# ZulutionAI/MoviiGen1.1

Measured on AMD Instinct MI355X. Metric: denoise-steps/sec, higher is better.
Workload: dtype bf16; 1 GPU; 14B T2V 1920x832x81f bf16 (the metric's configuration; BASELINE configs[2] shape); layers=40, parallelism=single, solver=unipc, weights=random N(0,0.02) bf16, seed 0

## Files before the change

moviigen1.1_amd/csrc/attn_hd128_m16.hip:

```cpp
#include <type_traits>
#include "common.h"
#include "../../include/moviigen_hip.h"

#define M16_THREADS 256
#define M16_QB 256
#define M16_TILE 16384
#define M16_K(slot) ((slot) * M16_TILE)
#define M16_V(slot) (3 * M16_TILE + (slot) * M16_TILE)

MG_DEV bf16x8_t m16_bf(u32x4_t v) { return __builtin_bit_cast(bf16x8_t, v); }
struct M16State {
    f32x4_t ot[8][4];
    f32x4_t st[2][2][4];
    bf16x8_t pf[2][4];
    f32x4_t mq[4];
    float m_run[4], l_run[4];
    float psa[4], psb[4];
    int bad;
};

template <int OFF>
MG_DEV void m16_rd(bf16x8_t& dst, unsigned addr) {
    asm volatile("ds_read_b128 %0, %1 offset:%2" : "=v"(dst) : "v"(addr), "i"(OFF));
}
template <int N>
MG_DEV void m16_wait() {
    asm volatile("s_waitcnt lgkmcnt(%0)" ::"i"(N) : "memory");
}
MG_DEV void m16_mfma_s0(f32x4_t& acc, const bf16x8_t& a, const bf16x8_t& b, const f32x4_t& c) {
    asm volatile("v_mfma_f32_16x16x32_bf16 %0, %1, %2, %3" : "=&v"(acc) : "v"(a), "a"(b), "v"(c));
}
MG_DEV void m16_mfma_s(f32x4_t& acc, const bf16x8_t& a, const bf16x8_t& b) {
    asm volatile("v_mfma_f32_16x16x32_bf16 %0, %1, %2, %0" : "+v"(acc) : "v"(a), "a"(b));
}
MG_DEV void m16_mfma_s_after_valu(f32x4_t& acc, const bf16x8_t& a, const bf16x8_t& b) {
    asm volatile("s_nop 7\n\ts_nop 7\n\tv_mfma_f32_16x16x32_bf16 %0, %1, %2, %0" : "+v"(acc) : "v"(a), "a"(b));
}
constexpr int m16_koff(int i) { return (i >> 2) * 256 + (i & 3) * 4096; }
constexpr int m16_voff(int i) { return i * 256; }

template <int KB>
MG_DEV void m16_softmax_exact(M16State& s, float c) {
#pragma unroll
    for (int n = 0; n < 4; ++n) {
        float tmax = s.st[KB][0][n][0];
#pragma unroll
        for (int r = 1; r < 4; ++r) tmax = fmaxf(tmax, s.st[KB][0][n][r]);
#pragma unroll
        for (int r = 0; r < 4; ++r) tmax = fmaxf(tmax, s.st[KB][1][n][r]);
        tmax = fmaxf(tmax, __shfl_xor(tmax, 16, 64));
        tmax = fmaxf(tmax, __shfl_xor(tmax, 32, 64));
        const float m_new = fmaxf(s.m_run[n], tmax);
        float psum = 0.f;
        float p[8];
#pragma unroll
        for (int r = 0; r < 8; ++r) {
            p[r] = __builtin_amdgcn_exp2f((s.st[KB][r >> 2][n][r & 3] - m_new) * c);
            psum += p[r];
        }
        u32x4_t w;
#pragma unroll
        for (int e = 0; e < 4; ++e) w[e] = pack_bf2(p[2 * e], p[2 * e + 1]);
        s.pf[KB][n] = m16_bf(w);
        const float alpha = __builtin_amdgcn_exp2f((s.m_run[n] - m_new) * c);
        s.l_run[n] = s.l_run[n] * alpha + psum;
#pragma unroll
        for (int d = 0; d < 8; ++d)
#pragma unroll
            for (int e = 0; e < 4; ++e) s.ot[d][n][e] *= alpha;
        s.m_run[n] = m_new;
    }
}

template <int KB>
MG_DEV void m16_softmax_zero(M16State& s, float c) {
#pragma unroll
    for (int n = 0; n < 4; ++n) {
        float psum = 0.f;
        float p[8];
#pragma unroll
        for (int r = 0; r < 8; ++r) {
            p[r] = __builtin_amdgcn_exp2f(s.st[KB][r >> 2][n][r & 3] * c);
            psum += p[r];
        }
        u32x4_t w;
#pragma unroll
        for (int e = 0; e < 4; ++e) w[e] = pack_bf2(p[2 * e], p[2 * e + 1]);
        s.pf[KB][n] = m16_bf(w);
        s.l_run[n] += psum;
    }
}

template <int KB>
MG_DEV void m16_mask_init(M16State& s, int lim, int G, const f32x4_t (&base)[4]) {
#pragma unroll
    for (int blk = 0; blk < 2; ++blk)
#pragma unroll
        for (int n = 0; n < 4; ++n)
#pragma unroll
            for (int r = 0; r < 4; ++r) {
                const int key = KB * 32 + G * 8 + blk * 4 + r;
                s.st[KB][blk][n][r] = key >= lim ? -1e30f : base[n][0];
            }
}

template <int KB, int SMODE, bool PV, bool SM, bool SCALED, int ORD, int LKO = 0, int LVO = 0, int NKO = 0, int NVO = 0, typename Dma>
MG_DEV void m16_step(M16State& s, const bf16x8_t (&qf)[4][4], bf16x8_t (&kf)[4], bf16x8_t (&vf)[4], unsigned lds_k,
                     unsigned lds_v, unsigned nk, unsigned nv, float c, Dma dma) {
    constexpr int SB = 1 - KB;
    u32x4_t w[4];
    float pa[2] = {0.f, 0.f}, pb[2] = {0.f, 0.f};
    auto exp_a = [&](int i, int half) __attribute__((always_inline)) {
        if (SM) {
            const int pp = 2 * i + half, n = pp >> 2, wd = pp & 3;
            const float x = s.st[SB][wd >> 1][n][(wd & 1) * 2];
            pa[half] = __builtin_amdgcn_exp2f(SCALED ? x * c : x);
            asm volatile("" : "+v"(pa[half]));
        }
    };
    auto exp_b = [&](int i, int half) __attribute__((always_inline)) {
        if (SM) {
            const int pp = 2 * i + half, n = pp >> 2, wd = pp & 3;
            const float x = s.st[SB][wd >> 1][n][(wd & 1) * 2 + 1];
            pb[half] = __builtin_amdgcn_exp2f(SCALED ? x * c : x);
            asm volatile("" : "+v"(pb[half]));
        }
    };
    auto add_a = [&](int i, int half) __attribute__((always_inline)) {
        if (SM) {
            const int n = (2 * i + half) >> 2;
            s.psa[n] += pa[half];
            asm volatile("" : "+v"(s.psa[n]));
        }
    };
    auto add_b = [&](int i, int half) __attribute__((always_inline)) {
        if (SM) {
            const int n = (2 * i + half) >> 2;
            s.psb[n] += pb[half];
            asm volatile("" : "+v"(s.psb[n]));
        }
    };
    auto cvt = [&](int i, int half) __attribute__((always_inline)) {
        if (SM) {
            const int pp = 2 * i + half, n = pp >> 2, wd = pp & 3;
            unsigned pk = pack_bf2(pa[half], pb[half]);
            asm volatile("" : "+v"(pk));
            w[n][wd] = pk;
        }
    };
    auto S = [&](int i, int n) __attribute__((always_inline)) {
        const int blk = i >> 2, c = i & 3, r = i & 3;
        if (SMODE == 1 && c == 0) m16_mfma_s0(s.st[KB][blk][n], kf[r], qf[n][c], s.mq[n]);
        else if (SMODE == 2 && c == 0) m16_mfma_s_after_valu(s.st[KB][blk][n], kf[r], qf[n][c]);
        else if (SMODE != 0) m16_mfma_s(s.st[KB][blk][n], kf[r], qf[n][c]);
    };
    auto P = [&](int i, int n) __attribute__((always_inline)) {
        if (PV) s.ot[i][n] = __builtin_amdgcn_mfma_f32_16x16x32_bf16(vf[i & 3], s.pf[KB][n], s.ot[i][n], 0, 0, 0);
    };
    auto rdK = [&](int i) __attribute__((always_inline)) {
        const int r2 = (i + 2) & 3;
        if (SMODE == 0) asm volatile("" ::"v"(kf[r2]));
        if (i < 6) {
            switch (i) {
                case 0: m16_rd<m16_koff(2) + LKO>(kf[r2], lds_k); break;
                case 1: m16_rd<m16_koff(3) + LKO>(kf[r2], lds_k); break;
                case 2: m16_rd<m16_koff(4) + LKO>(kf[r2], lds_k); break;
                case 3: m16_rd<m16_koff(5) + LKO>(kf[r2], lds_k); break;
                case 4: m16_rd<m16_koff(6) + LKO>(kf[r2], lds_k); break;
                default: m16_rd<m16_koff(7) + LKO>(kf[r2], lds_k); break;
            }
        } else if (i == 6) m16_rd<m16_koff(0) + NKO>(kf[r2], nk);
        else m16_rd<m16_koff(1) + NKO>(kf[r2], nk);
    };
    auto rdV = [&](int i) __attribute__((always_inline)) {
        const int r2 = (i + 2) & 3;
        if (i < 6) {
            switch (i) {
                case 0: m16_rd<m16_voff(2) + LVO>(vf[r2], lds_v); break;
                case 1: m16_rd<m16_voff(3) + LVO>(vf[r2], lds_v); break;
                case 2: m16_rd<m16_voff(4) + LVO>(vf[r2], lds_v); break;
                case 3: m16_rd<m16_voff(5) + LVO>(vf[r2], lds_v); break;
                case 4: m16_rd<m16_voff(6) + LVO>(vf[r2], lds_v); break;
                default: m16_rd<m16_voff(7) + LVO>(vf[r2], lds_v); break;
            }
        } else if (i == 6) m16_rd<m16_voff(0) + NVO>(vf[r2], nv);
        else m16_rd<m16_voff(1) + NVO>(vf[r2], nv);
    };
#define M16_SB() __builtin_amdgcn_sched_barrier(0)
#pragma unroll
    for (int i = 0; i < 8; ++i) {
        m16_wait<2>();
        M16_SB();
        if constexpr (ORD == 0) {
            S(i, 0); M16_SB();
            exp_a(i, 0); exp_b(i, 0); M16_SB();
            P(i, 0); M16_SB();
            add_a(i, 0); add_b(i, 0); cvt(i, 0); M16_SB();
            S(i, 1); M16_SB();
            rdK(i); M16_SB();
            P(i, 1); M16_SB();
            rdV(i); M16_SB();
            S(i, 2); M16_SB();
            exp_a(i, 1); exp_b(i, 1); M16_SB();
            P(i, 2); M16_SB();
            add_a(i, 1); add_b(i, 1); cvt(i, 1); M16_SB();
            S(i, 3); M16_SB();
            dma(i); M16_SB();
            P(i, 3); M16_SB();
        } else if constexpr (ORD == 1) {
            S(i, 0); M16_SB();
            exp_a(i, 0); M16_SB();
            P(i, 0); M16_SB();
            exp_b(i, 0); M16_SB();
            S(i, 1); M16_SB();
            add_a(i, 0); add_b(i, 0); cvt(i, 0); M16_SB();
            P(i, 1); M16_SB();
            rdK(i); M16_SB(); rdV(i); M16_SB();
            S(i, 2); M16_SB();
            exp_a(i, 1); M16_SB();
            P(i, 2); M16_SB();
            exp_b(i, 1); M16_SB();
            S(i, 3); M16_SB();
            add_a(i, 1); add_b(i, 1); cvt(i, 1); M16_SB();
            P(i, 3); M16_SB();
            dma(i); M16_SB();
        } else if constexpr (ORD == 2) {
            S(i, 0); M16_SB();
            exp_a(i, 0); M16_SB(); rdK(i); M16_SB();
            P(i, 0); M16_SB();
            exp_b(i, 0); M16_SB(); rdV(i); M16_SB();
            S(i, 1); M16_SB();
            add_a(i, 0); add_b(i, 0); cvt(i, 0); M16_SB();
            P(i, 1); M16_SB();
            S(i, 2); M16_SB();
            exp_a(i, 1); M16_SB();
            P(i, 2); M16_SB();
            exp_b(i, 1); M16_SB();
            S(i, 3); M16_SB();
            add_a(i, 1); add_b(i, 1); cvt(i, 1); M16_SB();
            P(i, 3); M16_SB();
            dma(i); M16_SB();
        } else if constexpr (ORD == 4) {
            S(i, 0); M16_SB();
            exp_a(i, 0); M16_SB();
            P(i, 0); M16_SB();
            exp_b(i, 0); M16_SB();
            S(i, 1); M16_SB();
            add_a(i, 0); add_b(i, 0); M16_SB();
            P(i, 1); M16_SB();
            cvt(i, 0); M16_SB(); rdK(i); M16_SB(); rdV(i); M16_SB();
            S(i, 2); M16_SB();
            exp_a(i, 1); M16_SB();
            P(i, 2); M16_SB();
            exp_b(i, 1); M16_SB();
            S(i, 3); M16_SB();
            add_a(i, 1); add_b(i, 1); M16_SB();
            P(i, 3); M16_SB();
            cvt(i, 1); M16_SB(); dma(i); M16_SB();
        } else if constexpr (ORD == 5) {
            S(i, 0); M16_SB();
            exp_a(i, 0); M16_SB();
            P(i, 0); M16_SB();
            exp_b(i, 0); M16_SB();
            S(i, 1); M16_SB();
            add_a(i, 0); add_b(i, 0); cvt(i, 0); M16_SB();
            P(i, 1); M16_SB();
            rdK(i); M16_SB();
            S(i, 2); M16_SB();
            exp_a(i, 1); M16_SB();
            P(i, 2); M16_SB();
            exp_b(i, 1); M16_SB();
            S(i, 3); M16_SB();
            add_a(i, 1); add_b(i, 1); cvt(i, 1); M16_SB();
            P(i, 3); M16_SB();
            rdV(i); M16_SB(); dma(i); M16_SB();
        } else if constexpr (ORD == 8) {
            S(i, 0); M16_SB();
            exp_a(i, 0); M16_SB();
            S(i, 1); M16_SB();
            exp_b(i, 0); M16_SB();
            P(i, 0); M16_SB();
            add_a(i, 0); add_b(i, 0); cvt(i, 0); M16_SB();
            P(i, 1); M16_SB();
            rdK(i); M16_SB(); rdV(i); M16_SB();
            S(i, 2); M16_SB();
            exp_a(i, 1); M16_SB();
            S(i, 3); M16_SB();
            exp_b(i, 1); M16_SB();
            P(i, 2); M16_SB();
            add_a(i, 1); add_b(i, 1); cvt(i, 1); M16_SB();
            P(i, 3); M16_SB();
            dma(i); M16_SB();
        } else if constexpr (ORD == 9) {
            S(i, 0); M16_SB();
            exp_a(i, 0); M16_SB();
            S(i, 1); M16_SB();
            exp_b(i, 0); M16_SB();
            S(i, 2); M16_SB();
            add_a(i, 0); add_b(i, 0); cvt(i, 0); M16_SB();
            S(i, 3); M16_SB();
            rdK(i); M16_SB(); rdV(i); M16_SB();
            P(i, 0); M16_SB();
            exp_a(i, 1); M16_SB();
            P(i, 1); M16_SB();
            exp_b(i, 1); M16_SB();
            P(i, 2); M16_SB();
            add_a(i, 1); add_b(i, 1); cvt(i, 1); M16_SB();
            P(i, 3); M16_SB();
            dma(i); M16_SB();
        } else {
            S(i, 0); M16_SB();
            exp_a(i, 0); M16_SB();
            P(i, 0); M16_SB();
            exp_b(i, 0); M16_SB();
            S(i, 1); M16_SB();
            exp_a(i, 1); M16_SB();
            P(i, 1); M16_SB();
            exp_b(i, 1); M16_SB();
            S(i, 2); M16_SB();
            add_a(i, 0); add_b(i, 0); cvt(i, 0); M16_SB();
            P(i, 2); M16_SB();
            add_a(i, 1); add_b(i, 1); cvt(i, 1); M16_SB();
            S(i, 3); M16_SB();
            rdK(i); M16_SB(); rdV(i); M16_SB();
            P(i, 3); M16_SB();
            dma(i); M16_SB();
        }
    }
#undef M16_SB
    if (SM) {
#pragma unroll
        for (int n = 0; n < 4; ++n) {
            s.pf[SB][n] = m16_bf(w[n]);
        }
    }
}

MG_DEV int m16_lane() {
    int l;
    asm volatile("v_mbcnt_lo_u32_b32 %0, -1, 0\n\tv_mbcnt_hi_u32_b32 %0, -1, %0" : "=v"(l));
    return l;
}

struct M16NoDma {
    __device__ __forceinline__ void operator()(int) const {}
};

template <bool PROF, bool SCALED, int ORD>
__global__ __launch_bounds__(M16_THREADS, 1) void attn_hd128_m16_kernel(
    const uint16_t* __restrict__ q, int64_t ldq, const uint16_t* __restrict__ kp, const uint16_t* __restrict__ vp,
    uint16_t* __restrict__ o, int64_t ldo, int64_t Lq, int64_t Lk, int heads, float c_log2, int nqb, int dbg,
    unsigned long long* __restrict__ prof, float* __restrict__ lse, unsigned* __restrict__ flagcnt, unsigned* __restrict__ tickets) {
    __shared__ __attribute__((aligned(16))) char smem[6 * M16_TILE];
    __shared__ int s_next_item;
    const int bid = blockIdx.x;
    const unsigned long long r_start = PROF ? __builtin_amdgcn_s_memrealtime() : 0;
    const int tid = threadIdx.x;
    const int wave = __builtin_amdgcn_readfirstlane(tid >> 6);
    const int total_items = nqb * heads;
    const int nwg = gridDim.x;
    const bool ticketed = tickets != nullptr && nwg != total_items;
    int item, item_end, item_step;
    if (nwg == total_items || ticketed) {
        item = bid, item_end = ticketed ? total_items : bid + 1, item_step = 1;
    } else {
        const int xcd = bid & 7, slot = bid >> 3;
        item = (int)((int64_t)xcd * total_items / 8) + slot;
        item_end = (int)((int64_t)(xcd + 1) * total_items / 8);
        item_step = nwg >> 3;
    }
    unsigned next_ticket = 0;
    unsigned long long ph[8] = {0, 0, 0, 0, 0, 0, 0, 0}, ph_t = 0;
    unsigned long long pf_fence = 0, pf_a = 0, pf_b = 0, pf_n = 0;
    while (item < item_end) {
    if (ticketed && tid == 0) next_ticket = atomicAdd(tickets, 1u);
    const int head = item / nqb;
    const int qb0 = item - head * nqb;
    const int lane = m16_lane();
    int qi = lane & 15, G = lane >> 4;
    __syncthreads();
    if (PROF) ph_t = __builtin_amdgcn_s_memtime();

    bf16x8_t qf[4][4];
    const int64_t qrow_base = (int64_t)qb0 * M16_QB + wave * 64 + qi;
#pragma unroll
    for (int n = 0; n < 4; ++n) {
        const int64_t qr = qrow_base + n * 16;
        const int64_t qrow = qr < Lq ? qr : Lq - 1;
        const uint16_t* qp = q + qrow * ldq + head * 128 + G * 8;
#pragma unroll
        for (int c = 0; c < 4; ++c) qf[n][c] = m16_bf(*(const u32x4_t*)(qp + c * 32));
    }
    const int T = (int)((Lk + 63) / 64);
    const int last_lim = (int)(Lk - (int64_t)(T - 1) * 64);
    const int nfull = last_lim == 64 ? T : T - 1;
    const unsigned lds0 = (unsigned)(uintptr_t)(mg_lptr_t)smem;
    const uint64_t kb64 = (uint64_t)(uintptr_t)(kp + ((int64_t)head * T) * 8192), vb64 = (uint64_t)(uintptr_t)(vp + ((int64_t)head * T) * 8192);
    const u32x4_t rs_k = {(unsigned)__builtin_amdgcn_readfirstlane((int)(unsigned)kb64), (unsigned)__builtin_amdgcn_readfirstlane((int)((unsigned)(kb64 >> 32) & 0xffffu)),
                          (unsigned)T * M16_TILE, 0x00020000u};
    const u32x4_t rs_v = {(unsigned)__builtin_amdgcn_readfirstlane((int)(unsigned)vb64), (unsigned)__builtin_amdgcn_readfirstlane((int)((unsigned)(vb64 >> 32) & 0xffffu)),
                          (unsigned)T * M16_TILE, 0x00020000u};
    const int dvo = wave * 4096 + lane * 16;
    const unsigned lds_w = (unsigned)__builtin_amdgcn_readfirstlane((int)(lds0 + wave * 4096));
    auto dma_tile4 = [&](const u32x4_t& rs, int t, unsigned lbase) __attribute__((always_inline)) {
        const int soff = __builtin_amdgcn_readfirstlane((t < T ? t : T - 1) * M16_TILE);
        asm volatile("s_mov_b32 m0, %2\n\ts_nop 4\n\t"
                     "buffer_load_dwordx4 %0, %1, %3 offen lds\n\t"
                     "buffer_load_dwordx4 %0, %1, %3 offen offset:1024 lds\n\t"
                     "buffer_load_dwordx4 %0, %1, %3 offen offset:2048 lds\n\t"
                     "buffer_load_dwordx4 %0, %1, %3 offen offset:3072 lds"
                     :: "v"(dvo), "s"(rs), "s"(lbase), "s"(soff) : "memory");
    };
    auto dma_k4 = [&](int t, int slot) __attribute__((always_inline)) { dma_tile4(rs_k, t, lds_w + M16_K(slot)); };
    auto dma_v4 = [&](int t, int slot) __attribute__((always_inline)) { dma_tile4(rs_v, t, lds_w + M16_V(slot)); };
    unsigned kbase = lds0 + G * 1024 + qi * 16;
    unsigned vbase = lds0 + 3 * M16_TILE + G * 2048 + qi * 16;
    auto k_addr = [&](int slot, int kb) __attribute__((always_inline)) { return kbase + slot * M16_TILE + kb * 512; };
    auto v_addr = [&](int slot, int kb) __attribute__((always_inline)) { return vbase + slot * M16_TILE + kb * 8192; };

    M16State s;
    bf16x8_t kf[4], vf[4];
    auto reset = [&]() __attribute__((always_inline)) {
#pragma unroll
        for (int d = 0; d < 8; ++d)
#pragma unroll
            for (int n = 0; n < 4; ++n) s.ot[d][n] = (f32x4_t){0.f, 0.f, 0.f, 0.f};
#pragma unroll
        for (int n = 0; n < 4; ++n) s.m_run[n] = -1e30f, s.l_run[n] = 0.f, s.psa[n] = 0.f, s.psb[n] = 0.f;
        s.bad = 0;
    };
    reset();
    auto q_pin = [&]() __attribute__((always_inline)) {
#pragma unroll
        for (int n = 0; n < 4; ++n)
#pragma unroll
            for (int c = 0; c < 4; ++c) asm volatile("" : "+a"(qf[n][c]));
    };
    auto fence = [&]() __attribute__((always_inline)) {
        asm volatile("s_waitcnt vmcnt(0)" ::: "memory");
        __syncthreads();
    };
    auto fence_hot = [&]() __attribute__((always_inline)) {
        asm volatile("s_waitcnt vmcnt(0)\n\ts_barrier" ::: "memory");
    };
    auto prefetch = [&](unsigned ak, unsigned av) __attribute__((always_inline)) {
        m16_rd<m16_koff(0)>(kf[0], ak);
        m16_rd<m16_voff(0)>(vf[0], av);
        m16_rd<m16_koff(1)>(kf[1], ak);
        m16_rd<m16_voff(1)>(vf[1], av);
    };
    const f32x4_t zero4[4] = {{0.f, 0.f, 0.f, 0.f}, {0.f, 0.f, 0.f, 0.f}, {0.f, 0.f, 0.f, 0.f}, {0.f, 0.f, 0.f, 0.f}};
    auto bare_S = [&](auto kbc, int slot, int lim) __attribute__((always_inline)) {
        constexpr int KB = decltype(kbc)::value;
        if (lim < 64) m16_mask_init<KB>(s, lim, G, zero4);
        else {
#pragma unroll
            for (int blk = 0; blk < 2; ++blk)
#pragma unroll
                for (int n = 0; n < 4; ++n) s.st[KB][blk][n] = (f32x4_t){0.f, 0.f, 0.f, 0.f};
        }
        const char* base = smem + M16_K(slot) + G * 1024 + qi * 16 + KB * 512;
#pragma unroll
        for (int i = 0; i < 8; ++i) {
            const bf16x8_t f = *(const bf16x8_t*)(base + m16_koff(i));
#pragma unroll
            for (int n = 0; n < 4; ++n)
                s.st[KB][i >> 2][n] = __builtin_amdgcn_mfma_f32_16x16x32_bf16(f, qf[n][i & 3], s.st[KB][i >> 2][n], 0, 0, 0);
        }
    };
    auto bare_PV = [&](auto kbc, int slot) __attribute__((always_inline)) {
        constexpr int KB = decltype(kbc)::value;
        const char* base = smem + M16_V(slot) + G * 2048 + qi * 16 + KB * 8192;
#pragma unroll
        for (int i = 0; i < 8; ++i) {
            const bf16x8_t f = *(const bf16x8_t*)(base + m16_voff(i));
#pragma unroll
            for (int n = 0; n < 4; ++n)
                s.ot[i][n] = __builtin_amdgcn_mfma_f32_16x16x32_bf16(f, s.pf[KB][n], s.ot[i][n], 0, 0, 0);
        }
    };
    using KB0 = std::integral_constant<int, 0>;
    using KB1 = std::integral_constant<int, 1>;

    bool exact_pass = nfull < 3;
    if (!exact_pass) {
    for (int attempt = 0;; ++attempt) {
        auto tile_max = [&](float (&mx)[4]) __attribute__((always_inline)) {
#pragma unroll
            for (int n = 0; n < 4; ++n) {
                float a = fmaxf(fmaxf(s.st[0][0][n][0], s.st[0][0][n][1]), fmaxf(s.st[0][0][n][2], s.st[0][0][n][3]));
                float b = fmaxf(fmaxf(s.st[0][1][n][0], s.st[0][1][n][1]), fmaxf(s.st[0][1][n][2], s.st[0][1][n][3]));
                float c2 = fmaxf(fmaxf(s.st[1][0][n][0], s.st[1][0][n][1]), fmaxf(s.st[1][0][n][2], s.st[1][0][n][3]));
                float d2 = fmaxf(fmaxf(s.st[1][1][n][0], s.st[1][1][n][1]), fmaxf(s.st[1][1][n][2], s.st[1][1][n][3]));
                mx[n] = fmaxf(mx[n], fmaxf(fmaxf(a, b), fmaxf(c2, d2)));
            }
        };
        auto set_reference = [&](const float (&mx)[4], float above) __attribute__((always_inline)) {
#pragma unroll
            for (int n = 0; n < 4; ++n) {
                float m = fmaxf(mx[n], __shfl_xor(mx[n], 16, 64));
                m = fmaxf(m, __shfl_xor(m, 32, 64)) + above;
                s.mq[n] = (f32x4_t){-m, -m, -m, -m};
            }
        };
        if (attempt) {
            float mx[4] = {-1e30f, -1e30f, -1e30f, -1e30f};
#pragma unroll
            for (int a = 0; a < 4; ++a) dma_k4(a, a);
            for (int t = 0; t < T; ++t) {
                asm volatile("s_waitcnt vmcnt(12)" ::: "memory");
                __syncthreads();
                dma_k4(t + 4, (t + 4) % 6);
                const int lim = t == T - 1 ? last_lim : 64;
                bare_S(KB0{}, t % 6, lim);
                bare_S(KB1{}, t % 6, lim);
                tile_max(mx);
            }
            asm volatile("s_waitcnt vmcnt(0)" ::: "memory");
            set_reference(mx, 0.f);
            __syncthreads();
            reset();
        }
        dma_k4(0, 0), dma_v4(0, 0), dma_k4(1, 1);
        fence();
        q_pin();
        if (PROF) { const unsigned long long tt = __builtin_amdgcn_s_memtime(); ph[0] += tt - ph_t; ph_t = tt; }
        dma_k4(2, 2), dma_v4(1, 1);
        bare_S(KB0{}, 0, 64);
        bare_S(KB1{}, 0, 64);
        if (attempt == 0) {
            float mx[4] = {-1e30f, -1e30f, -1e30f, -1e30f};
            tile_max(mx);
            set_reference(mx, c_log2 > 1e-20f ? 64.f / c_log2 : 0.f);
        }
#pragma unroll
        for (int kb = 0; kb < 2; ++kb)
#pragma unroll
            for (int blk = 0; blk < 2; ++blk)
#pragma unroll
                for (int n = 0; n < 4; ++n) s.st[kb][blk][n] += s.mq[n];
        m16_softmax_zero<0>(s, c_log2);
#pragma unroll
        for (int n = 0; n < 4; ++n) asm volatile("" : "+v"(s.l_run[n]));
        prefetch(k_addr(1, 0), v_addr(0, 0));
        m16_step<0, 1, true, true, SCALED, ORD>(s, qf, kf, vf, k_addr(1, 0), v_addr(0, 0), k_addr(1, 1), v_addr(0, 1), c_log2, M16NoDma());
        int t = 1;
        unsigned ka0 = k_addr(0, 0), ka1 = k_addr(1, 0), ka2 = k_addr(2, 0);
        unsigned va0 = v_addr(0, 0), va1 = v_addr(1, 0), va2 = v_addr(2, 0);
        unsigned lk0 = (unsigned)__builtin_amdgcn_readfirstlane((int)(lds0 + M16_K(0) + wave * 4096));
        unsigned lk1 = lk0 + M16_TILE, lk2 = lk0 + 2 * M16_TILE;
        int offk = (t + 2) * M16_TILE, offv = (t + 1) * M16_TILE;
        unsigned keep_m0, rot_tmp;
#define M16_BDMA0(VOFF, RS, SOFF, LBASE, IMM)                                                                                              \
    asm volatile("s_add_u32 m0, %2, %3\n\ts_nop 0\n\tbuffer_load_dwordx4 %0, %1, %4 offen lds"                                             \
                 :: "v"(VOFF), "s"(RS), "s"(LBASE), "n"(IMM), "s"(SOFF) : "memory", "scc")
#define M16_BDMAN(VOFF, RS, SOFF, IMM)                                                                                                     \
    asm volatile("buffer_load_dwordx4 %0, %1, %3 offen offset:%2 lds" :: "v"(VOFF), "s"(RS), "n"(IMM), "s"(SOFF) : "memory")
        asm volatile("s_mov_b32 %0, m0\n\ts_nop 4" : "=s"(keep_m0) :: "memory");
        if (PROF) { const unsigned long long tt = __builtin_amdgcn_s_memtime(); ph[1] += tt - ph_t; ph_t = tt; }
        __builtin_amdgcn_s_waitcnt(0x0F70);
        asm volatile("" : "+v"(ka0), "+v"(ka1), "+v"(ka2), "+v"(va0), "+v"(va1), "+v"(va2));
        if (PROF) { const unsigned long long tt = __builtin_amdgcn_s_memtime(); ph[2] += tt - ph_t; ph_t = tt; }
        for (; t + 1 < nfull; ++t) {
            const unsigned long long c0 = PROF ? __builtin_amdgcn_s_memtime() : 0;
            fence_hot();
            const unsigned long long c1 = PROF ? __builtin_amdgcn_s_memtime() : 0;
            m16_step<1, 1, true, true, SCALED, ORD, 512, 8192, 0, 0>(s, qf, kf, vf, ka1, va0, ka2, va1, c_log2,
                                       [&](int n) __attribute__((always_inline)) {
                                           switch (n) {
                                               case 0: M16_BDMA0(dvo, rs_k, offk, lk0, 0); break;
                                               case 1: M16_BDMAN(dvo, rs_k, offk, 1024); break;
                                               case 2: M16_BDMAN(dvo, rs_k, offk, 2048); break;
                                               case 3: M16_BDMAN(dvo, rs_k, offk, 3072); break;
                                               case 4: M16_BDMA0(dvo, rs_v, offv, lk2, 3 * M16_TILE); break;
                                               case 5: M16_BDMAN(dvo, rs_v, offv, 1024); break;
                                               case 6: M16_BDMAN(dvo, rs_v, offv, 2048); break;
                                               default: M16_BDMAN(dvo, rs_v, offv, 3072); break;
                                           }
                                       });
            const unsigned long long c2 = PROF ? __builtin_amdgcn_s_memtime() : 0;
            m16_step<0, 1, true, true, SCALED, ORD, 0, 0, 512, 8192>(s, qf, kf, vf, ka2, va1, ka2, va1, c_log2,
                                       [&](int n) __attribute__((always_inline)) {
                                           if (n == 0)
                                               asm volatile("s_add_u32 %0, %0, 0x4000\n\ts_add_u32 %1, %1, 0x4000" : "+s"(offk), "+s"(offv) : : "scc");
                                           else if (n == 1)
                                               asm volatile("s_mov_b32 %3, %0\n\ts_mov_b32 %0, %1\n\ts_mov_b32 %1, %2\n\ts_mov_b32 %2, %3"
                                                            : "+s"(lk0), "+s"(lk1), "+s"(lk2), "=&s"(rot_tmp));
                                           else if (n == 7) {
                                               asm volatile("v_swap_b32 %0, %1\n\tv_swap_b32 %1, %2" : "+v"(ka0), "+v"(ka1), "+v"(ka2));
                                               asm volatile("v_swap_b32 %0, %1\n\tv_swap_b32 %1, %2" : "+v"(va0), "+v"(va1), "+v"(va2));
                                           }
                                       });
            if (PROF) {
                const unsigned long long c3 = __builtin_amdgcn_s_memtime();
                pf_fence += c1 - c0, pf_a += c2 - c1, pf_b += c3 - c2, pf_n += 1;
            }
        }
#undef M16_BDMA0
#undef M16_BDMAN
        asm volatile("s_mov_b32 m0, %0" :: "s"(keep_m0) : "memory");
        if (PROF) { const unsigned long long tt = __builtin_amdgcn_s_memtime(); ph[3] += tt - ph_t; ph_t = tt; }
        static_assert(M16_TILE == 0x4000, "the literal above");
        const int s0 = (t - 1) % 3, s1 = t % 3, s2 = (t + 1) % 3;
        {
            const int l2 = m16_lane();
            qi = l2 & 15, G = l2 >> 4;
            kbase = lds0 + G * 1024 + qi * 16;
            vbase = lds0 + 3 * M16_TILE + G * 2048 + qi * 16;
        }
        fence();
        if (t + 1 < T) {
            dma_v4(t + 1, s2);
        }
        m16_step<1, 1, true, true, SCALED, ORD>(s, qf, kf, vf, k_addr(s1, 1), v_addr(s0, 1), k_addr(s2, 0), v_addr(s1, 0), c_log2, M16NoDma());
        if (t + 1 < T) {
            m16_mask_init<0>(s, last_lim, G, s.mq);
            m16_step<0, 2, true, true, SCALED, ORD>(s, qf, kf, vf, k_addr(s2, 0), v_addr(s1, 0), k_addr(s2, 1), v_addr(s1, 1), c_log2, M16NoDma());
            fence();
            m16_mask_init<1>(s, last_lim, G, s.mq);
            m16_step<1, 2, true, true, SCALED, ORD>(s, qf, kf, vf, k_addr(s2, 1), v_addr(s1, 1), k_addr(s2, 1), v_addr(s2, 0), c_log2, M16NoDma());
            m16_step<0, 0, true, true, SCALED, ORD>(s, qf, kf, vf, k_addr(s2, 1), v_addr(s2, 0), k_addr(s2, 1), v_addr(s2, 1), c_log2, M16NoDma());
            m16_step<1, 0, true, false, SCALED, ORD>(s, qf, kf, vf, k_addr(s2, 1), v_addr(s2, 1), k_addr(s2, 1), v_addr(s2, 1), c_log2, M16NoDma());
        } else {
            m16_step<0, 0, true, true, SCALED, ORD>(s, qf, kf, vf, k_addr(s1, 1), v_addr(s1, 0), k_addr(s1, 1), v_addr(s1, 1), c_log2, M16NoDma());
            m16_step<1, 0, true, false, SCALED, ORD>(s, qf, kf, vf, k_addr(s1, 1), v_addr(s1, 1), k_addr(s1, 1), v_addr(s1, 1), c_log2, M16NoDma());
        }
        m16_wait<0>();
        asm volatile("" ::"v"(kf[0]), "v"(kf[1]), "v"(kf[2]), "v"(kf[3]), "v"(vf[0]), "v"(vf[1]), "v"(vf[2]), "v"(vf[3]));
#pragma unroll
        for (int n = 0; n < 4; ++n) {
            s.l_run[n] += s.psa[n] + s.psb[n];
            s.psa[n] = s.psb[n] = 0.f;
            float lt = s.l_run[n] + __shfl_xor(s.l_run[n], 16, 64);
            lt += __shfl_xor(lt, 32, 64);
            s.bad |= !(lt >= 8.4703295e-22f && lt <= 1.2379400e27f);
            s.m_run[n] = -s.mq[n][0];
        }
        const bool flagged = __syncthreads_or(s.bad) != 0;
        if (PROF) { const unsigned long long tt = __builtin_amdgcn_s_memtime(); ph[4] += tt - ph_t; ph_t = tt; }
        if (!flagged || (dbg & 1)) break;
        if (flagcnt && tid == 0) atomicAdd(flagcnt + (attempt ? 1 : 0), 1u);
        if (attempt) {
            exact_pass = true;
            break;
        }
    }
    }
    if (exact_pass) {
        reset();
        for (int t = 0; t < T; ++t) {
            __syncthreads();
            dma_k4(t, 0), dma_v4(t, 0);
            fence();
            q_pin();
            const int lim = t == T - 1 ? last_lim : 64;
            bare_S(KB0{}, 0, lim);
            bare_S(KB1{}, 0, lim);
            m16_softmax_exact<0>(s, c_log2);
            bare_PV(KB0{}, 0);
            m16_softmax_exact<1>(s, c_log2);
            bare_PV(KB1{}, 0);
        }
    }

    {
        const int l3 = m16_lane();
        qi = l3 & 15, G = l3 >> 4;
    }
#pragma unroll
    for (int n = 0; n < 4; ++n) {
        float l_tot = s.l_run[n] + __shfl_xor(s.l_run[n], 16, 64);
        l_tot += __shfl_xor(l_tot, 32, 64);
        const float inv = 1.f / l_tot;
        const int64_t qr = (int64_t)qb0 * M16_QB + wave * 64 + n * 16 + qi;
        if (lse && G == 0 && qr < Lq) lse[(int64_t)head * Lq + qr] = (s.m_run[n] * c_log2 + __log2f(l_tot)) * 0.6931471805599453f;
        if (qr < Lq) {
            uint16_t* op = o + qr * ldo + head * 128 + G * 4;
#pragma unroll
            for (int d = 0; d < 8; ++d) {
                uint2 pk;
                pk.x = pack_bf2(s.ot[d][n][0] * inv, s.ot[d][n][1] * inv);
                pk.y = pack_bf2(s.ot[d][n][2] * inv, s.ot[d][n][3] * inv);
                *(uint2*)(op + d * 16) = pk;
            }
        }
    }
    if (PROF) { ph[7] += __builtin_amdgcn_s_memtime() - ph_t; asm volatile("s_waitcnt vmcnt(0)" ::: "memory"); const unsigned long long tt = __builtin_amdgcn_s_memtime(); ph[5] += tt - ph_t; ph[6] += 1; }
    if (ticketed) {
        if (tid == 0) s_next_item = nwg + (int)next_ticket;
        __syncthreads();
        item = __builtin_amdgcn_readfirstlane(s_next_item);
    } else
        item += item_step;
    }
    if (ticketed && tid == 0 && atomicAdd(tickets + 1, 1u) == (unsigned)nwg - 1) {
        __hip_atomic_store(tickets, 0u, __ATOMIC_RELAXED, __HIP_MEMORY_SCOPE_AGENT);
        __hip_atomic_store(tickets + 1, 0u, __ATOMIC_RELAXED, __HIP_MEMORY_SCOPE_AGENT);
    }
    if (PROF && prof && tid == 0) prof[16 + 2 * bid] = r_start, prof[16 + 2 * bid + 1] = __builtin_amdgcn_s_memrealtime();
    if (PROF && prof && (tid & 63) == 0) {
        atomicAdd(prof + wave * 4 + 0, pf_fence);
        atomicAdd(prof + wave * 4 + 1, pf_a);
        atomicAdd(prof + wave * 4 + 2, pf_b);
        atomicAdd(prof + wave * 4 + 3, pf_n);
    }
    if (PROF && prof && tid == 0) {
#pragma unroll
        for (int i = 0; i < 8; ++i) atomicAdd(prof + 1040 + i, ph[i]);
    }
}

static int g_m16_dbg = 0;
static unsigned long long* g_m16_prof = nullptr;
static unsigned* g_m16_flagcnt = nullptr;
void mg_attn_m16_hooks(int dbg, unsigned long long* prof, unsigned* flagcnt) { g_m16_dbg = dbg, g_m16_prof = prof, g_m16_flagcnt = flagcnt; }

int mg_attn_m16_launch(const uint16_t* q, int64_t ldq, const uint16_t* kp, const uint16_t* vp, uint16_t* o, int64_t ldo,
                       int64_t Lq, int64_t Lk, int heads, float c_log2, int prescaled, int nqb, float* lse, int reserve_cus,
                       unsigned* workspace, hipStream_t st) {
    const int n_cu = mg_persistent_cus(reserve_cus);
    if (n_cu < 0) return MG_ERR_LAUNCH;
    const int total = nqb * heads;
    const unsigned grid = total <= n_cu ? (unsigned)total : (unsigned)n_cu;
    unsigned* tickets = nullptr;
    if (workspace && (int64_t)total >= 32 * (int64_t)grid && !(g_m16_dbg & 16))
        tickets = workspace;
#define M16_ORD 9
#define M16_LAUNCH(PROF, SCALED, ORD)                                                                                             \
    hipLaunchKernelGGL((attn_hd128_m16_kernel<PROF, SCALED, ORD>), dim3(grid), dim3(M16_THREADS), 0, st, q, ldq, kp, vp, o, ldo, Lq, \
                       Lk, heads, prescaled ? 1.0f : c_log2, nqb, g_m16_dbg, PROF ? g_m16_prof : nullptr, lse, g_m16_flagcnt, tickets)
#ifdef MG_AB_BUILD
    const int ord = (g_m16_dbg >> 1) & 7;
    const int mo = (g_m16_dbg >> 5) & 3;
    if (mo && prescaled && !g_m16_prof) {
        if (mo == 1) M16_LAUNCH(false, false, 8);
        else if (mo == 2) M16_LAUNCH(false, false, 9);
        else M16_LAUNCH(false, false, 1);
        return mg_check_launch();
    }
    if (ord && prescaled && !g_m16_prof) {
        if (ord == 1) M16_LAUNCH(false, false, 1);
        else if (ord == 2) M16_LAUNCH(false, false, 2);
        else if (ord == 3) M16_LAUNCH(false, false, 3);
        else if (ord == 4) M16_LAUNCH(false, false, 4);
        else if (ord == 5) M16_LAUNCH(false, false, 5);
        else M16_LAUNCH(false, false, 0);
        return mg_check_launch();
    }
#endif
    if (g_m16_prof) {
        if (prescaled) M16_LAUNCH(true, false, M16_ORD);
        else M16_LAUNCH(true, true, M16_ORD);
    } else {
        if (prescaled) M16_LAUNCH(false, false, M16_ORD);
        else M16_LAUNCH(false, true, M16_ORD);
    }
#undef M16_LAUNCH
    return mg_check_launch();
}
```

Before: 0.04579 steps/s.

## Add five-query-block-per-wave attention variant selected by a work-rounds cost rule

Templates the HD128 flash-attention kernel state and loops on the number of 16-row query blocks per wave, so a wave can hold 5 blocks (320 queries per work item) as well as the previous 4 (256). The 5-block variant gets its own hand-scheduled MFMA, exp and LDS-read interleave. A host-side rule compares the number of persistent-grid rounds for each item size, weighted by a per-item cost ratio that depends on Lk, and picks one. The intent is to reuse each loaded K/V tile across more query rows and cut tail rounds. In exchange each wave holds more accumulator registers and runs a different instruction schedule.

```diff
diff --git a/moviigen1.1_amd/csrc/attn_hd128_m16.hip b/moviigen1.1_amd/csrc/attn_hd128_m16.hip
--- a/moviigen1.1_amd/csrc/attn_hd128_m16.hip
+++ b/moviigen1.1_amd/csrc/attn_hd128_m16.hip
@@ -1,21 +1,23 @@
 #include <type_traits>
 #include "common.h"
 #include "../../include/moviigen_hip.h"
+#include "attn_m16_rule.h"
 
 #define M16_THREADS 256
-#define M16_QB 256
+#define M16_ITEM(NQ) (64 * (NQ))
 #define M16_TILE 16384
 #define M16_K(slot) ((slot) * M16_TILE)
 #define M16_V(slot) (3 * M16_TILE + (slot) * M16_TILE)
 
 MG_DEV bf16x8_t m16_bf(u32x4_t v) { return __builtin_bit_cast(bf16x8_t, v); }
+template <int NQ>
 struct M16State {
-    f32x4_t ot[8][4];
-    f32x4_t st[2][2][4];
-    bf16x8_t pf[2][4];
-    f32x4_t mq[4];
-    float m_run[4], l_run[4];
-    float psa[4], psb[4];
+    f32x4_t ot[8][NQ];
+    f32x4_t st[2][2][NQ];
+    bf16x8_t pf[2][NQ];
+    f32x4_t mq[NQ];
+    float m_run[NQ], l_run[NQ];
+    float psa[NQ], psb[NQ];
     int bad;
 };
 
@@ -39,10 +41,10 @@
 constexpr int m16_koff(int i) { return (i >> 2) * 256 + (i & 3) * 4096; }
 constexpr int m16_voff(int i) { return i * 256; }
 
-template <int KB>
-MG_DEV void m16_softmax_exact(M16State& s, float c) {
-#pragma unroll
-    for (int n = 0; n < 4; ++n) {
+template <int KB, int NQ>
+MG_DEV void m16_softmax_exact(M16State<NQ>& s, float c) {
+#pragma unroll
+    for (int n = 0; n < NQ; ++n) {
         float tmax = s.st[KB][0][n][0];
 #pragma unroll
         for (int r = 1; r < 4; ++r) tmax = fmaxf(tmax, s.st[KB][0][n][r]);
@@ -72,10 +74,10 @@
     }
 }
 
-template <int KB>
-MG_DEV void m16_softmax_zero(M16State& s, float c) {
-#pragma unroll
-    for (int n = 0; n < 4; ++n) {
+template <int KB, int NQ>
+MG_DEV void m16_softmax_zero(M16State<NQ>& s, float c) {
+#pragma unroll
+    for (int n = 0; n < NQ; ++n) {
         float psum = 0.f;
         float p[8];
 #pragma unroll
@@ -91,12 +93,12 @@
     }
 }
 
-template <int KB>
-MG_DEV void m16_mask_init(M16State& s, int lim, int G, const f32x4_t (&base)[4]) {
+template <int KB, int NQ>
+MG_DEV void m16_mask_init(M16State<NQ>& s, int lim, int G, const f32x4_t (&base)[NQ]) {
 #pragma unroll
     for (int blk = 0; blk < 2; ++blk)
 #pragma unroll
-        for (int n = 0; n < 4; ++n)
+        for (int n = 0; n < NQ; ++n)
 #pragma unroll
             for (int r = 0; r < 4; ++r) {
                 const int key = KB * 32 + G * 8 + blk * 4 + r;
@@ -104,15 +106,15 @@
             }
 }
 
-template <int KB, int SMODE, bool PV, bool SM, bool SCALED, int ORD, int LKO = 0, int LVO = 0, int NKO = 0, int NVO = 0, typename Dma>
-MG_DEV void m16_step(M16State& s, const bf16x8_t (&qf)[4][4], bf16x8_t (&kf)[4], bf16x8_t (&vf)[4], unsigned lds_k,
+template <int KB, int SMODE, bool PV, bool SM, bool SCALED, int ORD, int LKO = 0, int LVO = 0, int NKO = 0, int NVO = 0, int NQ, typename Dma>
+MG_DEV void m16_step(M16State<NQ>& s, const bf16x8_t (&qf)[NQ][4], bf16x8_t (&kf)[4], bf16x8_t (&vf)[4], unsigned lds_k,
                      unsigned lds_v, unsigned nk, unsigned nv, float c, Dma dma) {
     constexpr int SB = 1 - KB;
-    u32x4_t w[4];
-    float pa[2] = {0.f, 0.f}, pb[2] = {0.f, 0.f};
+    u32x4_t w[NQ];
+    float pa[NQ - 2] = {0.f, 0.f}, pb[NQ - 2] = {0.f, 0.f};
     auto exp_a = [&](int i, int half) __attribute__((always_inline)) {
         if (SM) {
-            const int pp = 2 * i + half, n = pp >> 2, wd = pp & 3;
+            const int pp = NQ * i / 2 + half, n = pp >> 2, wd = pp & 3;
             const float x = s.st[SB][wd >> 1][n][(wd & 1) * 2];
             pa[half] = __builtin_amdgcn_exp2f(SCALED ? x * c : x);
             asm volatile("" : "+v"(pa[half]));
@@ -120,7 +122,7 @@
     };
     auto exp_b = [&](int i, int half) __attribute__((always_inline)) {
         if (SM) {
-            const int pp = 2 * i + half, n = pp >> 2, wd = pp & 3;
+            const int pp = NQ * i / 2 + half, n = pp >> 2, wd = pp & 3;
             const float x = s.st[SB][wd >> 1][n][(wd & 1) * 2 + 1];
             pb[half] = __builtin_amdgcn_exp2f(SCALED ? x * c : x);
             asm volatile("" : "+v"(pb[half]));
@@ -128,21 +130,21 @@
     };
     auto add_a = [&](int i, int half) __attribute__((always_inline)) {
         if (SM) {
-            const int n = (2 * i + half) >> 2;
+            const int n = (NQ * i / 2 + half) >> 2;
             s.psa[n] += pa[half];
             asm volatile("" : "+v"(s.psa[n]));
         }
     };
     auto add_b = [&](int i, int half) __attribute__((always_inline)) {
         if (SM) {
-            const int n = (2 * i + half) >> 2;
+            const int n = (NQ * i / 2 + half) >> 2;
             s.psb[n] += pb[half];
             asm volatile("" : "+v"(s.psb[n]));
         }
     };
     auto cvt = [&](int i, int half) __attribute__((always_inline)) {
         if (SM) {
-            const int pp = 2 * i + half, n = pp >> 2, wd = pp & 3;
+            const int pp = NQ * i / 2 + half, n = pp >> 2, wd = pp & 3;
             unsigned pk = pack_bf2(pa[half], pb[half]);
             asm volatile("" : "+v"(pk));
             w[n][wd] = pk;
@@ -191,7 +193,50 @@
     for (int i = 0; i < 8; ++i) {
         m16_wait<2>();
         M16_SB();
-        if constexpr (ORD == 0) {
+        if constexpr (NQ == 5) {
+            static_assert(ORD == 9, "five query blocks per wave exist in the shipped order only");
+            if ((i & 1) == 0) {
+                S(i, 0); M16_SB();
+                exp_a(i, 0); M16_SB();
+                S(i, 1); M16_SB();
+                exp_b(i, 0); M16_SB();
+                S(i, 2); M16_SB();
+                add_a(i, 0); add_b(i, 0); cvt(i, 0); M16_SB();
+                S(i, 3); M16_SB();
+                S(i, 4); M16_SB();
+                rdK(i); M16_SB(); rdV(i); M16_SB();
+                P(i, 0); M16_SB();
+                exp_a(i, 1); M16_SB();
+                P(i, 1); M16_SB();
+                exp_b(i, 1); M16_SB();
+                P(i, 2); M16_SB();
+                add_a(i, 1); add_b(i, 1); cvt(i, 1); M16_SB();
+                P(i, 3); M16_SB();
+                P(i, 4); M16_SB();
+                dma(i); M16_SB();
+            } else {
+                S(i, 0); M16_SB();
+                exp_a(i, 0); M16_SB();
+                S(i, 1); M16_SB();
+                exp_b(i, 0); M16_SB();
+                S(i, 2); M16_SB();
+                add_a(i, 0); add_b(i, 0); cvt(i, 0); M16_SB();
+                S(i, 3); M16_SB();
+                exp_a(i, 1); M16_SB();
+                S(i, 4); M16_SB();
+                exp_b(i, 1); M16_SB();
+                P(i, 0); M16_SB();
+                add_a(i, 1); add_b(i, 1); cvt(i, 1); M16_SB();
+                P(i, 1); M16_SB();
+                exp_a(i, 2); M16_SB();
+                P(i, 2); M16_SB();
+                exp_b(i, 2); M16_SB();
+                P(i, 3); M16_SB();
+                add_a(i, 2); add_b(i, 2); cvt(i, 2); M16_SB();
+                P(i, 4); M16_SB();
+                rdK(i); M16_SB(); rdV(i); M16_SB(); dma(i); M16_SB();
+            }
+        } else if constexpr (ORD == 0) {
             S(i, 0); M16_SB();
             exp_a(i, 0); exp_b(i, 0); M16_SB();
             P(i, 0); M16_SB();
@@ -330,7 +375,7 @@
 #undef M16_SB
     if (SM) {
 #pragma unroll
-        for (int n = 0; n < 4; ++n) {
+        for (int n = 0; n < NQ; ++n) {
             s.pf[SB][n] = m16_bf(w[n]);
         }
     }
@@ -346,7 +391,7 @@
     __device__ __forceinline__ void operator()(int) const {}
 };
 
-template <bool PROF, bool SCALED, int ORD>
+template <bool PROF, bool SCALED, int ORD, int NQ>
 __global__ __launch_bounds__(M16_THREADS, 1) void attn_hd128_m16_kernel(
     const uint16_t* __restrict__ q, int64_t ldq, const uint16_t* __restrict__ kp, const uint16_t* __restrict__ vp,
     uint16_t* __restrict__ o, int64_t ldo, int64_t Lq, int64_t Lk, int heads, float c_log2, int nqb, int dbg,
@@ -381,10 +426,10 @@
     __syncthreads();
     if (PROF) ph_t = __builtin_amdgcn_s_memtime();
 
-    bf16x8_t qf[4][4];
-    const int64_t qrow_base = (int64_t)qb0 * M16_QB + wave * 64 + qi;
-#pragma unroll
-    for (int n = 0; n < 4; ++n) {
+    bf16x8_t qf[NQ][4];
+    const int64_t qrow_base = (int64_t)qb0 * M16_ITEM(NQ) + wave * (16 * NQ) + qi;
+#pragma unroll
+    for (int n = 0; n < NQ; ++n) {
         const int64_t qr = qrow_base + n * 16;
         const int64_t qrow = qr < Lq ? qr : Lq - 1;
         const uint16_t* qp = q + qrow * ldq + head * 128 + G * 8;
@@ -418,21 +463,21 @@
     auto k_addr = [&](int slot, int kb) __attribute__((always_inline)) { return kbase + slot * M16_TILE + kb * 512; };
     auto v_addr = [&](int slot, int kb) __attribute__((always_inline)) { return vbase + slot * M16_TILE + kb * 8192; };
 
-    M16State s;
+    M16State<NQ> s;
     bf16x8_t kf[4], vf[4];
     auto reset = [&]() __attribute__((always_inline)) {
 #pragma unroll
         for (int d = 0; d < 8; ++d)
 #pragma unroll
-            for (int n = 0; n < 4; ++n) s.ot[d][n] = (f32x4_t){0.f, 0.f, 0.f, 0.f};
-#pragma unroll
-        for (int n = 0; n < 4; ++n) s.m_run[n] = -1e30f, s.l_run[n] = 0.f, s.psa[n] = 0.f, s.psb[n] = 0.f;
+            for (int n = 0; n < NQ; ++n) s.ot[d][n] = (f32x4_t){0.f, 0.f, 0.f, 0.f};
+#pragma unroll
+        for (int n = 0; n < NQ; ++n) s.m_run[n] = -1e30f, s.l_run[n] = 0.f, s.psa[n] = 0.f, s.psb[n] = 0.f;
         s.bad = 0;
     };
     reset();
     auto q_pin = [&]() __attribute__((always_inline)) {
 #pragma unroll
-        for (int n = 0; n < 4; ++n)
+        for (int n = 0; n < NQ; ++n)
 #pragma unroll
             for (int c = 0; c < 4; ++c) asm volatile("" : "+a"(qf[n][c]));
     };
@@ -449,7 +494,7 @@
         m16_rd<m16_koff(1)>(kf[1], ak);
         m16_rd<m16_voff(1)>(vf[1], av);
     };
-    const f32x4_t zero4[4] = {{0.f, 0.f, 0.f, 0.f}, {0.f, 0.f, 0.f, 0.f}, {0.f, 0.f, 0.f, 0.f}, {0.f, 0.f, 0.f, 0.f}};
+    const f32x4_t zero4[NQ] = {{0.f, 0.f, 0.f, 0.f}, {0.f, 0.f, 0.f, 0.f}, {0.f, 0.f, 0.f, 0.f}, {0.f, 0.f, 0.f, 0.f}};
     auto bare_S = [&](auto kbc, int slot, int lim) __attribute__((always_inline)) {
         constexpr int KB = decltype(kbc)::value;
         if (lim < 64) m16_mask_init<KB>(s, lim, G, zero4);
@@ -457,14 +502,14 @@
 #pragma unroll
             for (int blk = 0; blk < 2; ++blk)
 #pragma unroll
-                for (int n = 0; n < 4; ++n) s.st[KB][blk][n] = (f32x4_t){0.f, 0.f, 0.f, 0.f};
+                for (int n = 0; n < NQ; ++n) s.st[KB][blk][n] = (f32x4_t){0.f, 0.f, 0.f, 0.f};
         }
         const char* base = smem + M16_K(slot) + G * 1024 + qi * 16 + KB * 512;
 #pragma unroll
         for (int i = 0; i < 8; ++i) {
             const bf16x8_t f = *(const bf16x8_t*)(base + m16_koff(i));
 #pragma unroll
-            for (int n = 0; n < 4; ++n)
+            for (int n = 0; n < NQ; ++n)
                 s.st[KB][i >> 2][n] = __builtin_amdgcn_mfma_f32_16x16x32_bf16(f, qf[n][i & 3], s.st[KB][i >> 2][n], 0, 0, 0);
         }
     };
@@ -475,7 +520,7 @@
         for (int i = 0; i < 8; ++i) {
             const bf16x8_t f = *(const bf16x8_t*)(base + m16_voff(i));
 #pragma unroll
-            for (int n = 0; n < 4; ++n)
+            for (int n = 0; n < NQ; ++n)
                 s.ot[i][n] = __builtin_amdgcn_mfma_f32_16x16x32_bf16(f, s.pf[KB][n], s.ot[i][n], 0, 0, 0);
         }
     };
@@ -485,9 +530,9 @@
     bool exact_pass = nfull < 3;
     if (!exact_pass) {
     for (int attempt = 0;; ++attempt) {
-        auto tile_max = [&](float (&mx)[4]) __attribute__((always_inline)) {
-#pragma unroll
-            for (int n = 0; n < 4; ++n) {
+        auto tile_max = [&](float (&mx)[NQ]) __attribute__((always_inline)) {
+#pragma unroll
+            for (int n = 0; n < NQ; ++n) {
                 float a = fmaxf(fmaxf(s.st[0][0][n][0], s.st[0][0][n][1]), fmaxf(s.st[0][0][n][2], s.st[0][0][n][3]));
                 float b = fmaxf(fmaxf(s.st[0][1][n][0], s.st[0][1][n][1]), fmaxf(s.st[0][1][n][2], s.st[0][1][n][3]));
                 float c2 = fmaxf(fmaxf(s.st[1][0][n][0], s.st[1][0][n][1]), fmaxf(s.st[1][0][n][2], s.st[1][0][n][3]));
@@ -495,16 +540,17 @@
                 mx[n] = fmaxf(mx[n], fmaxf(fmaxf(a, b), fmaxf(c2, d2)));
             }
         };
-        auto set_reference = [&](const float (&mx)[4], float above) __attribute__((always_inline)) {
-#pragma unroll
-            for (int n = 0; n < 4; ++n) {
+        auto set_reference = [&](const float (&mx)[NQ], float above) __attribute__((always_inline)) {
+#pragma unroll
+            for (int n = 0; n < NQ; ++n) {
                 float m = fmaxf(mx[n], __shfl_xor(mx[n], 16, 64));
                 m = fmaxf(m, __shfl_xor(m, 32, 64)) + above;
                 s.mq[n] = (f32x4_t){-m, -m, -m, -m};
             }
         };
         if (attempt) {
-            float mx[4] = {-1e30f, -1e30f, -1e30f, -1e30f};
+            float mx[NQ] = {-1e30f, -1e30f, -1e30f, -1e30f};
+            mx[NQ - 1] = -1e30f;
 #pragma unroll
             for (int a = 0; a < 4; ++a) dma_k4(a, a);
             for (int t = 0; t < T; ++t) {
@@ -529,7 +575,8 @@
         bare_S(KB0{}, 0, 64);
         bare_S(KB1{}, 0, 64);
         if (attempt == 0) {
-            float mx[4] = {-1e30f, -1e30f, -1e30f, -1e30f};
+            float mx[NQ] = {-1e30f, -1e30f, -1e30f, -1e30f};
+            mx[NQ - 1] = -1e30f;
             tile_max(mx);
             set_reference(mx, c_log2 > 1e-20f ? 64.f / c_log2 : 0.f);
         }
@@ -538,10 +585,10 @@
 #pragma unroll
             for (int blk = 0; blk < 2; ++blk)
 #pragma unroll
-                for (int n = 0; n < 4; ++n) s.st[kb][blk][n] += s.mq[n];
+                for (int n = 0; n < NQ; ++n) s.st[kb][blk][n] += s.mq[n];
         m16_softmax_zero<0>(s, c_log2);
 #pragma unroll
-        for (int n = 0; n < 4; ++n) asm volatile("" : "+v"(s.l_run[n]));
+        for (int n = 0; n < NQ; ++n) asm volatile("" : "+v"(s.l_run[n]));
         prefetch(k_addr(1, 0), v_addr(0, 0));
         m16_step<0, 1, true, true, SCALED, ORD>(s, qf, kf, vf, k_addr(1, 0), v_addr(0, 0), k_addr(1, 1), v_addr(0, 1), c_log2, M16NoDma());
         int t = 1;
@@ -628,7 +675,7 @@
         m16_wait<0>();
         asm volatile("" ::"v"(kf[0]), "v"(kf[1]), "v"(kf[2]), "v"(kf[3]), "v"(vf[0]), "v"(vf[1]), "v"(vf[2]), "v"(vf[3]));
 #pragma unroll
-        for (int n = 0; n < 4; ++n) {
+        for (int n = 0; n < NQ; ++n) {
             s.l_run[n] += s.psa[n] + s.psb[n];
             s.psa[n] = s.psb[n] = 0.f;
             float lt = s.l_run[n] + __shfl_xor(s.l_run[n], 16, 64);
@@ -668,11 +715,11 @@
         qi = l3 & 15, G = l3 >> 4;
     }
 #pragma unroll
-    for (int n = 0; n < 4; ++n) {
+    for (int n = 0; n < NQ; ++n) {
         float l_tot = s.l_run[n] + __shfl_xor(s.l_run[n], 16, 64);
         l_tot += __shfl_xor(l_tot, 32, 64);
         const float inv = 1.f / l_tot;
-        const int64_t qr = (int64_t)qb0 * M16_QB + wave * 64 + n * 16 + qi;
+        const int64_t qr = (int64_t)qb0 * M16_ITEM(NQ) + wave * (16 * NQ) + n * 16 + qi;
         if (lse && G == 0 && qr < Lq) lse[(int64_t)head * Lq + qr] = (s.m_run[n] * c_log2 + __log2f(l_tot)) * 0.6931471805599453f;
         if (qr < Lq) {
             uint16_t* op = o + qr * ldo + head * 128 + G * 4;
@@ -720,15 +767,23 @@
                        unsigned* workspace, hipStream_t st) {
     const int n_cu = mg_persistent_cus(reserve_cus);
     if (n_cu < 0) return MG_ERR_LAUNCH;
+    int item_q = mg_attn_m16_item_queries(Lq, Lk, heads, n_cu);
+#ifdef MG_AB_BUILD
+    const int force_nq = (g_m16_dbg >> 7) & 3;
+    if (force_nq) item_q = force_nq == 2 ? 320 : 256;
+    if ((g_m16_dbg & 0x6e) != 0) item_q = 256;
+#endif
+    if (item_q != 256) nqb = (int)((Lq + item_q - 1) / item_q);
     const int total = nqb * heads;
     const unsigned grid = total <= n_cu ? (unsigned)total : (unsigned)n_cu;
     unsigned* tickets = nullptr;
     if (workspace && (int64_t)total >= 32 * (int64_t)grid && !(g_m16_dbg & 16))
         tickets = workspace;
 #define M16_ORD 9
-#define M16_LAUNCH(PROF, SCALED, ORD)                                                                                             \
-    hipLaunchKernelGGL((attn_hd128_m16_kernel<PROF, SCALED, ORD>), dim3(grid), dim3(M16_THREADS), 0, st, q, ldq, kp, vp, o, ldo, Lq, \
+#define M16_LAUNCH_NQ(PROF, SCALED, ORD, NQ)                                                                                      \
+    hipLaunchKernelGGL((attn_hd128_m16_kernel<PROF, SCALED, ORD, NQ>), dim3(grid), dim3(M16_THREADS), 0, st, q, ldq, kp, vp, o, ldo, Lq, \
                        Lk, heads, prescaled ? 1.0f : c_log2, nqb, g_m16_dbg, PROF ? g_m16_prof : nullptr, lse, g_m16_flagcnt, tickets)
+#define M16_LAUNCH(PROF, SCALED, ORD) M16_LAUNCH_NQ(PROF, SCALED, ORD, 4)
 #ifdef MG_AB_BUILD
     const int ord = (g_m16_dbg >> 1) & 7;
     const int mo = (g_m16_dbg >> 5) & 3;
@@ -748,7 +803,15 @@
         return mg_check_launch();
     }
 #endif
-    if (g_m16_prof) {
+    if (item_q == 320) {
+        if (g_m16_prof) {
+            if (prescaled) M16_LAUNCH_NQ(true, false, M16_ORD, 5);
+            else M16_LAUNCH_NQ(true, true, M16_ORD, 5);
+        } else {
+            if (prescaled) M16_LAUNCH_NQ(false, false, M16_ORD, 5);
+            else M16_LAUNCH_NQ(false, true, M16_ORD, 5);
+        }
+    } else if (g_m16_prof) {
         if (prescaled) M16_LAUNCH(true, false, M16_ORD);
         else M16_LAUNCH(true, true, M16_ORD);
     } else {
@@ -756,5 +819,6 @@
         else M16_LAUNCH(false, true, M16_ORD);
     }
 #undef M16_LAUNCH
+#undef M16_LAUNCH_NQ
     return mg_check_launch();
 }
diff --git a/moviigen1.1_amd/csrc/attn_m16_rule.h b/moviigen1.1_amd/csrc/attn_m16_rule.h
--- /dev/null
+++ b/moviigen1.1_amd/csrc/attn_m16_rule.h
@@ -0,0 +1,26 @@
+#pragma once
+#include <cstdint>
+
+#define MG_M16_RULE_RHO 1.210
+#define MG_M16_RULE_FIXED_TILES 15.0
+#define MG_M16_RULE_FIXED_TILES_5 46.0
+#define MG_M16_RULE_MIN_ROUNDS 32
+
+static inline int64_t mg_attn_m16_items(int64_t Lq, int heads, int item_queries) {
+    return (Lq + item_queries - 1) / item_queries * heads;
+}
+static inline int64_t mg_attn_m16_grid(int64_t items, int n_cu) { return items <= n_cu ? items : n_cu; }
+static inline int64_t mg_attn_m16_rounds(int64_t items, int n_cu) {
+    const int64_t g = mg_attn_m16_grid(items, n_cu);
+    return g > 0 ? (items + g - 1) / g : 0;
+}
+static inline double mg_attn_m16_item_ratio(int64_t Lk) {
+    const double T = (double)((Lk + 63) / 64);
+    return (MG_M16_RULE_FIXED_TILES_5 + MG_M16_RULE_RHO * T) / (MG_M16_RULE_FIXED_TILES + T);
+}
+static inline int mg_attn_m16_item_queries(int64_t Lq, int64_t Lk, int heads, int n_cu) {
+    if (Lq <= 0 || Lk <= 0 || heads <= 0 || n_cu <= 0) return 256;
+    const int64_t items5 = mg_attn_m16_items(Lq, heads, 320), items4 = mg_attn_m16_items(Lq, heads, 256);
+    if (items5 < MG_M16_RULE_MIN_ROUNDS * mg_attn_m16_grid(items5, n_cu)) return 256;
+    return (double)mg_attn_m16_rounds(items5, n_cu) * mg_attn_m16_item_ratio(Lk) < (double)mg_attn_m16_rounds(items4, n_cu) ? 320 : 256;
+}
```

Result: no change. 0.04611 steps/s (median of 6 runs) (+0.7%).
